# kezakool/flair-for-aigle

Measured on AMD Instinct MI355X. Metric: 512x512x5 tiles/sec (train fwd+bwd+AdamW), U-Net ResNet-34, 19 classes, higher is better.
Workload: dtype bf16; 1 GPU; synthetic 512x512x5 tiles, 19-class U-Net (ResNet-34 encoder), batch 32 per GPU, train step (BASELINE.json configs[1]); global_batch=32, tile=512, parallelism=dp1

## Files before the change

### flair-for-aigle_amd/csrc/conv_igemm.hip

```cpp
#include "ffa_gfx950.h"

#include <stdlib.h>

#ifndef FFA_CONV_READS_FIRST
#define FFA_CONV_READS_FIRST 0
#endif

#ifndef FFA_CONV_TRACE
#define FFA_CONV_TRACE 0
#endif
#if FFA_CONV_TRACE
#ifndef FFA_CONV_TRACE_FIRST
#define FFA_CONV_TRACE_FIRST 0
#endif
__device__ long long ffa_conv_trace_buf[64 * 256];
#define FFA_TRACE(slot_)                                                                    \
  if (trace_on) {                                                                           \
    if (trace_n < 256) ffa_conv_trace_buf[(blockIdx.x - FFA_CONV_TRACE_FIRST) * 256 + trace_n] = (long long)(slot_) << 56 | (__builtin_readcyclecounter() & 0xFFFFFFFFFFFFFFLL); \
    ++trace_n;                                                                              \
  }
#else
#define FFA_TRACE(slot_)
#endif

// ... 647 lines not shown
      const bool ok = (i < G::H_PIECES) && vy >= 0 && vx >= 0 && vy < a.Hi && vx < a.Wi;
      ho[k] = ok ? (((t.b * a.Hi + vy) * a.Wi + vx) * a.Ci * EB + hh * 16) : -1;
    }
  };

  int vb = next_valid(blockIdx.x);
  if (vb >= total_vb) return;
  TileId cur = decode(vb);
  int hoff[G::NHP];
  halo_offsets(cur, hoff);
  const unsigned char* in_b = static_cast<const unsigned char*>(a.in);
  const unsigned char* w_all = static_cast<const unsigned char*>(a.w);
  const unsigned char* w_b = w_all + (size_t)cur.cb * total_chunks * slab;

  ffa_u32x4 wregA[G::NWP], wregB[G::NWP];
  ffa_u32x4 hreg[G::NHP];
  ffa_f32x16 acc[G::MT][G::NT];

#define FFA_P_STORE_W(WR)                                                                  \
  {                                                                                        \
    _Pragma("unroll") for (int k = 0; k < G::NWP; ++k) {                                   \
      const int i = tid + k * G::NTHR;                                                     \
      if (k + 1 < G::NWP || G::W_PIECES % G::NTHR == 0 || i < G::W_PIECES) {               \
        const int row = i / (G::TAPS * 2), col = i % (G::TAPS * 2);                        \
        *reinterpret_cast<ffa_u32x4*>(sW + row * G::WP + col * 16) = WR[k];                \
      }                                                                                    \
    }                                                                                      \
  }
#define FFA_P_STORE_H(HO)                                                                  \
  {                                                                                        \
    _Pragma("unroll") for (int k = 0; k < G::NHP; ++k) {                                   \
      const int i = tid + k * G::NTHR;                                                     \
      if (k + 1 < G::NHP || G::H_PIECES % G::NTHR == 0 || i < G::H_PIECES)                 \
        *reinterpret_cast<ffa_u32x4*>(sIn + hlds0 + k * HLDS_STEP) = (HO[k] >= 0) ? hreg[k] : ffa_u32x4{0u, 0u, 0u, 0u}; \
    }                                                                                      \
  }

  {
    const ffa_u32x4* wsrc = reinterpret_cast<const ffa_u32x4*>(w_b);
#pragma unroll
    for (int k = 0; k < G::NWP; ++k) {
      const int i = tid + k * G::NTHR;
      wregA[k] = wsrc[(k + 1 < G::NWP || G::W_PIECES % G::NTHR == 0 || i < G::W_PIECES) ? i : 0];
    }
#pragma unroll
    for (int k = 0; k < G::NHP; ++k) hreg[k] = *reinterpret_cast<const ffa_u32x4*>(in_b + (unsigned)(hoff[k] >= 0 ? hoff[k] : 0));
    FFA_P_STORE_W(wregA)
    FFA_P_STORE_H(hoff)
    __syncthreads();
    const ffa_u32x4* wsrc1 = reinterpret_cast<const ffa_u32x4*>(w_b + slab);
#pragma unroll
    for (int k = 0; k < G::NWP; ++k) {
      const int i = tid + k * G::NTHR;
      wregA[k] = wsrc1[(k + 1 < G::NWP || G::W_PIECES % G::NTHR == 0 || i < G::W_PIECES) ? i : 0];
    }
  }

  constexpr int HJ = (HK >= 4) ? 1 : 0;
  while (true) {
    const int nvb = next_valid(vb + gridDim.x);
    const bool has_next = nvb < total_vb;
    const TileId nxt = decode(has_next ? nvb : vb);
    const unsigned char* w_n = w_all + (size_t)nxt.cb * total_chunks * slab;

#pragma unroll
    for (int mt = 0; mt < G::MT; ++mt)
#pragma unroll
      for (int nt = 0; nt < G::NT; ++nt)
#pragma unroll
        for (int r = 0; r < 16; ++r) acc[mt][nt][r] = 0.f;

    for (int c0 = 0; c0 < total_chunks; c0 += HK) {
      const bool last_group = (c0 + HK >= total_chunks);
      const bool cross = last_group && has_next;
      const unsigned char* hbase = in_b + (last_group ? (has_next ? 0 : c0 * 32) : (c0 + HK) * 32);
      if (cross) halo_offsets(nxt, hoff);
#pragma unroll
      for (int j = 0; j < HK; ++j) {
        const int c = c0 + j;
        const unsigned char* wp = (c + 2 < total_chunks) ? w_b + (size_t)(c + 2) * slab
                                  : (has_next ? w_n + (size_t)(c + 2 - total_chunks) * slab
                                              : w_b + (size_t)(total_chunks - 1) * slab);
        const ffa_u32x4* wsrc = reinterpret_cast<const ffa_u32x4*>(wp);
        auto issue = [&](int tap) __attribute__((always_inline)) {
#pragma unroll
          for (int k = 0; k < G::NWP; ++k) {
            if (k % G::TAPS != tap) continue;
            const int i = tid + k * G::NTHR;
            const ffa_u32x4 v = wsrc[(k + 1 < G::NWP || G::W_PIECES % G::NTHR == 0 || i < G::W_PIECES) ? i : 0];
            if (j & 1) wregA[k] = v;
            else wregB[k] = v;
          }
          if (j == HJ) {
#pragma unroll
            for (int k = 0; k < G::NHP; ++k) {
              if (k % G::TAPS != tap) continue;
              hreg[k] = *reinterpret_cast<const ffa_u32x4*>(hbase + (unsigned)(hoff[k] >= 0 ? hoff[k] : 0));
            }
          }
        };
        {
          const int sub = j * 32;
          ffa_u32x4 af[2][G::MT], bf[2][G::NT];
#pragma unroll
          for (int mt = 0; mt < G::MT; ++mt) af[0][mt] = *reinterpret_cast<const ffa_u32x4*>(sW + aoff[mt]);
#pragma unroll
          for (int nt = 0; nt < G::NT; ++nt) bf[0][nt] = *reinterpret_cast<const ffa_u32x4*>(sIn + boff[nt] + sub);
#pragma unroll
          for (int tap = 0; tap < G::TAPS; ++tap) {
            const int cu = tap & 1, nx = cu ^ 1;
            __builtin_amdgcn_sched_barrier(0);
            issue(tap);
            if (tap + 1 < G::TAPS) {
              const int r1 = (tap + 1) / KW, s1 = (tap + 1) % KW;
#pragma unroll
              for (int mt = 0; mt < G::MT; ++mt)
                af[nx][mt] = *reinterpret_cast<const ffa_u32x4*>(sW + aoff[mt] + (tap + 1) * 32);
#pragma unroll
              for (int nt = 0; nt < G::NT; ++nt)
                bf[nx][nt] = *reinterpret_cast<const ffa_u32x4*>(sIn + boff[nt] + sub + (r1 * G::IW + s1) * G::PP);
            }
#pragma unroll
            for (int mt = 0; mt < G::MT; ++mt)
#pragma unroll
              for (int nt = 0; nt < G::NT; ++nt) Mma<T>::run(af[cu][mt], bf[cu][nt], acc[mt][nt]);
            {
              constexpr int NM = G::MT * G::NT;
              const int NR = (tap + 1 < G::TAPS) ? G::MT + G::NT : 0;
              int NV = 0;
#pragma unroll
              for (int k = 0; k < G::NWP; ++k) NV += (k % G::TAPS == tap) ? 1 : 0;
              if (j == HJ) {
#pragma unroll
                for (int k = 0; k < G::NHP; ++k) NV += (k % G::TAPS == tap) ? 1 : 0;
              }
              constexpr int PER = (sizeof(T) == 2) ? 1 : 4;
#pragma unroll
              for (int i = 0; i < NM; ++i) {
                __builtin_amdgcn_sched_group_barrier(0x008, PER, 0);
                if (i < NR) __builtin_amdgcn_sched_group_barrier(0x100, 1, 0);
                if (i < NV) __builtin_amdgcn_sched_group_barrier(0x020, 1, 0);
              }
#pragma unroll
              for (int i = NM; i < G::MT + G::NT; ++i)
                if (i < NR) __builtin_amdgcn_sched_group_barrier(0x100, 1, 0);
#pragma unroll
              for (int i = NM; i < NM + 4; ++i)
                if (i < NV) __builtin_amdgcn_sched_group_barrier(0x020, 1, 0);
            }
          }
          __builtin_amdgcn_sched_barrier(0);
        }
        __syncthreads();
        if (c + 1 < total_chunks || has_next) {
          if (j & 1) FFA_P_STORE_W(wregB)
          else FFA_P_STORE_W(wregA)
          if (j == HK - 1) FFA_P_STORE_H(hoff)
          __syncthreads();
        }
      }
    }

    {
      T* out = static_cast<T*>(a.out);
      const T* res = static_cast<const T*>(a.res);
      const int co_wave = cur.cb * BCO;
      constexpr int NCH = (G::MT == 2) ? 32 : 16;
      float st[2 * NCH];
      const bool want_stats = a.stats != nullptr;
#pragma unroll
      for (int i = 0; i < 2 * NCH; ++i) st[i] = 0.f;
#pragma unroll
      for (int nt = 0; nt < G::NT; ++nt) {
        const int n = wpx * G::WAVE_PX + nt * 32 + rho;
        const int oy = cur.oy0 + n / TW, ox = cur.ox0 + n % TW;
        if (oy >= a.Ho || ox >= a.Wo) continue;
        const long long pix = ((long long)(cur.b * a.Ho + oy) * a.Wo + ox) * (long long)a.Co;
#pragma unroll
        for (int g = 0; g < 4; ++g) {
          if (G::MT == 2) {
            const int c0 = co_wave + 16 * g + 8 * half;
            if (c0 >= a.Co) continue;
            float v[8];
#pragma unroll
            for (int i = 0; i < 4; ++i) {
              v[i] = acc[0][nt][4 * g + i];
              v[4 + i] = acc[G::MT - 1][nt][4 * g + i];
            }
            if (a.bias) {
#pragma unroll
              for (int i = 0; i < 8; ++i) v[i] += a.bias[c0 + i];
            }
            if (res) {
              float rv[8];
              ffa_load8<T>(res + pix + c0, rv);
#pragma unroll
              for (int i = 0; i < 8; ++i) v[i] += rv[i];
            }
            if (a.relu) {
#pragma unroll
              for (int i = 0; i < 8; ++i) v[i] = fmaxf(v[i], 0.f);
            }
            ffa_store8<T>(out + pix + c0, v);
            if (want_stats) {
#pragma unroll
              for (int i = 0; i < 8; ++i) {
                const float r = (EB == 2) ? ffa_bf16_bits_to_f32(ffa_f32_to_bf16_bits(v[i])) : v[i];
                st[g * 8 + i] += r;
                st[NCH + g * 8 + i] = __builtin_fmaf(r, r, st[NCH + g * 8 + i]);
              }
            }
          } else {
            const int c0 = co_wave + 8 * g + 4 * half;
            if (c0 >= a.Co) continue;
            float v[4];
#pragma unroll
            for (int i = 0; i < 4; ++i) v[i] = acc[0][nt][4 * g + i];
            if (a.bias) {
#pragma unroll
              for (int i = 0; i < 4; ++i) v[i] += a.bias[c0 + i];
            }
            if (res) {
#pragma unroll
              for (int i = 0; i < 4; ++i) v[i] += ffa_load_elem<T>(res + pix + c0 + i);
            }
            if (a.relu) {
#pragma unroll
              for (int i = 0; i < 4; ++i) v[i] = fmaxf(v[i], 0.f);
            }
            if (EB == 2) {
              uint2 u;
              u.x = ffa_pack_bf16x2(v[0], v[1]);
              u.y = ffa_pack_bf16x2(v[2], v[3]);
              *reinterpret_cast<uint2*>(out + pix + c0) = u;
            } else {
              *reinterpret_cast<float4*>(out + pix + c0) = make_float4(v[0], v[1], v[2], v[3]);
            }
            if (want_stats) {
#pragma unroll
              for (int i = 0; i < 4; ++i) {
                const float r = (EB == 2) ? ffa_bf16_bits_to_f32(ffa_f32_to_bf16_bits(v[i])) : v[i];
                st[g * 4 + i] += r;
                st[NCH + g * 4 + i] = __builtin_fmaf(r, r, st[NCH + g * 4 + i]);
              }
            }
          }
        }
      }
      if (want_stats) {
#pragma unroll
        for (int bit = 4; bit >= 0; --bit) {
          const int n = (2 * NCH) >> (4 - bit);
          if (n > 2) {
            const bool up = (rho >> bit) & 1;
#pragma unroll
            for (int jj = 0; jj < NCH; ++jj) {
              if (jj < n / 2) {
                float lo = st[jj], hi = st[jj + n / 2];
                asm volatile("" : "+v"(lo), "+v"(hi));
                const float keep = up ? hi : lo;
                const float send = up ? lo : hi;
                st[jj] = keep + __shfl_xor(send, 1 << bit, 64);
              }
            }
          } else {
            st[0] += __shfl_xor(st[0], 1 << bit, 64);
            st[1] += __shfl_xor(st[1], 1 << bit, 64);
          }
        }
        red[(wpx * 64 + lane) * 2 + 0] = st[0];
        red[(wpx * 64 + lane) * 2 + 1] = st[1];
        __syncthreads();
        constexpr int NOUT = (G::MT == 2) ? 128 : 64;
        if (tid < NOUT) {
          const int jj = tid & 1;
          const int ln = (G::MT == 2) ? (tid >> 1) : ((tid >> 1) * 2);
          float t = 0.f;
#pragma unroll
          for (int w = 0; w < WPX; ++w) t += red[(w * 64 + ln) * 2 + jj];
          const int r5 = ln & 31, hf = ln >> 5;
          const int which = r5 >> 4;
          int c;
          if (G::MT == 2) {
            const int L = (r5 & 15) * 2 + jj;
            c = cur.cb * BCO + 16 * (L >> 3) + 8 * hf + (L & 7);
          } else {
            const int L = ((r5 >> 1) & 7) * 2 + jj;
            c = cur.cb * BCO + 8 * (L >> 2) + 4 * hf + (L & 3);
          }
          if (c < a.Co) a.stats[((size_t)cur.pt * 2 + which) * a.Co + c] = t;
        }
        __syncthreads();
      }
    }
    if (!has_next) break;
    vb = nvb;
    cur = nxt;
    w_b = w_n;
  }
#undef FFA_P_STORE_W
#undef FFA_P_STORE_H
}


struct ConvPlan {
  int bco;
  int rg;
  int th, tw;
};

static int conv_rg(int kh) { return kh == 7 ? 1 : kh; }

static int conv_pref_bco(int kh, int kw, int stride, int cout) {
  if (kh == 3 && kw == 3 && stride == 1) return cout > 32 ? 64 : 32;
  return cout > 32 ? 64 : 32;
}

static bool conv_supported(int kh, int kw, int stride, int bco) {
  const bool shape = (kh == 3 && kw == 3 && (stride == 1 || stride == 2)) ||
                     (kh == 1 && kw == 1 && (stride == 1 || stride == 2)) || (kh == 7 && kw == 7 && stride == 2);
  if (!shape) return false;
  return bco == 64 || bco == 32;
}

static int conv_persist_grid(int dil, int c1_out, const void* bnx, int grid) {
  const char* pe = getenv("FFA_CONV_PERSIST");
  if ((pe && pe[0] == '0') || dil != 1 || c1_out != 0 || bnx != nullptr) return 0;
  const char* pm = getenv("FFA_CONV_PERSIST_MIN");
  const char* pg = getenv("FFA_CONV_PERSIST_GRID");
  const int min_grid = pm ? atoi(pm) : 0;
  int pgrid = pg ? atoi(pg) : 512;
  pgrid = pgrid < 8 ? 8 : (pgrid / 8) * 8;
  if (grid <= min_grid) return 0;
  return pgrid < grid ? pgrid : grid;
}

template <typename T, int KH, int KW, int STRIDE, int RG, int BCO, int WCO, int WPX, int TH, int TW, int HK,
          bool UP = false>
static int launch_hk(const ConvArgs& a, hipStream_t stream) {
  const int grid = ffa_cdiv(a.npt, 8) * 8 * a.ncb;
  if constexpr (KH == 3 && KW == 3 && STRIDE == 1 && HK >= 2 && !UP && WCO == 1 && WPX == 4) {
    const int pgrid = conv_persist_grid(a.dil, a.c1_out, a.bnx, grid);
    if (pgrid > 0) {
      hipLaunchKernelGGL((conv3x3_persist_kernel<T, BCO, TH, TW, HK>), dim3(pgrid), dim3(256), 0, stream, a);
      return ffa_check_launch("conv3x3_persist");
    }
  }
  hipLaunchKernelGGL((conv_igemm_kernel<T, KH, KW, STRIDE, RG, BCO, WCO, WPX, TH, TW, HK, UP>), dim3(grid),
                     dim3(64 * WCO * WPX), 0, stream, a);
  return ffa_check_launch("conv_igemm");
}

template <typename T, int BCO, int TH, int TW>
static int launch_up(const ConvArgs& a, hipStream_t stream) {
  if (a.nchunks % 4 == 0) return launch_hk<T, 3, 3, 1, 3, BCO, 1, 4, TH, TW, 4, true>(a, stream);
  return launch_hk<T, 3, 3, 1, 3, BCO, 1, 4, TH, TW, 2, true>(a, stream);
}

template <typename T, int KH, int KW, int STRIDE, int RG, int BCO, int WCO, int WPX, int TH, int TW>
static int launch_cfg(const ConvArgs& a, hipStream_t stream) {
  if constexpr (KH == 3 && STRIDE == 1) {
    if (a.nchunks % 4 == 0) return launch_hk<T, KH, KW, STRIDE, RG, BCO, WCO, WPX, TH, TW, 4>(a, stream);
    if (a.nchunks % 2 == 0) return launch_hk<T, KH, KW, STRIDE, RG, BCO, WCO, WPX, TH, TW, 2>(a, stream);
  }
  return launch_hk<T, KH, KW, STRIDE, RG, BCO, WCO, WPX, TH, TW, 1>(a, stream);
}

template <typename T, int KH, int KW, int STRIDE, int RG>
static int launch_shape(const ConvArgs& a, const ConvPlan& p, hipStream_t stream) {
  const bool wide = (p.tw == 32);
#define FFA_CONV_CASE(BCO_, WCO_, WPX_)                                                      \
  if (p.bco == BCO_) {                                                                       \
    return wide ? launch_cfg<T, KH, KW, STRIDE, RG, BCO_, WCO_, WPX_, 8, 32>(a, stream)      \
                : launch_cfg<T, KH, KW, STRIDE, RG, BCO_, WCO_, WPX_, 16, 16>(a, stream);    \
  }
  FFA_CONV_CASE(64, 1, 4)
  FFA_CONV_CASE(32, 1, 4)
#undef FFA_CONV_CASE
  ffa_set_error("conv: no kernel for bco=%d", p.bco);
  return FFA_ERR_UNSUPPORTED;
}

template <typename T>
static int launch_dtype(const ConvArgs& a, int kh, int kw, int stride, const ConvPlan& p, hipStream_t stream) {
  if (kh == 3 && kw == 3 && stride == 1) return launch_shape<T, 3, 3, 1, 3>(a, p, stream);
  if (kh == 3 && kw == 3 && stride == 2) return launch_shape<T, 3, 3, 2, 3>(a, p, stream);
  if (kh == 1 && kw == 1 && stride == 1) return launch_shape<T, 1, 1, 1, 1>(a, p, stream);
  if (kh == 1 && kw == 1 && stride == 2) return launch_shape<T, 1, 1, 2, 1>(a, p, stream);
  if (kh == 7 && kw == 7 && stride == 2) return launch_shape<T, 7, 7, 2, 1>(a, p, stream);
  ffa_set_error("conv: unsupported kernel %dx%d stride %d", kh, kw, stride);
  return FFA_ERR_UNSUPPORTED;
}

extern "C" int ffa_conv_block_co(int kh, int kw, int stride, int cout) {
  const int bco = conv_pref_bco(kh, kw, stride, cout);
  return conv_supported(kh, kw, stride, bco) ? bco : FFA_ERR_UNSUPPORTED;
}

extern "C" int ffa_conv_plan(int dtype, int kh, int kw, int stride, int cout, int ci_pitch, int allow_ring) {
  const int bco = ffa_conv_block_co(kh, kw, stride, cout);
  if (bco < 0) return bco;
  {
    const char* t = getenv("FFA_STEM");
    if ((allow_ring & 4) && !(t && t[0] == '0') && ffa_stem_eligible(dtype, kh, kw, stride, cout, ci_pitch))
      return 64 | FFA_BCO_STEM;
  }
  {
    const char* t = getenv("FFA_THIN");
    if ((allow_ring & 2) && !(t && t[0] == '0') && ffa_thin_eligible(dtype, kh, kw, stride, cout, ci_pitch))
      return (cout <= 16 ? 16 : 32) | FFA_BCO_THIN | (ci_pitch == 32 ? FFA_BCO_THIN32 : 0);
  }
  allow_ring &= 1;
  const char* e = getenv("FFA_RING");
  const int eb = (dtype == FFA_BF16) ? 2 : 4;
  const bool on = (dtype == FFA_BF16) ? !(e && e[0] == '0') : (e && e[0] == '1');
  if (allow_ring && on && kh == 3 && kw == 3 && stride == 1 && cout >= 64 && (ci_pitch * eb) % 64 == 0)
    return 64 | FFA_BCO_RING;
  return bco;
}

extern "C" int ffa_conv_row_group(int kh) { return conv_rg(kh); }

static int conv2d_impl(int dtype, const void* in, const void* w_packed, const float* bias, const void* residual,
                       void* out, float* stat_partials, int B, int Hi, int Wi, int Ci, int Ho, int Wo, int Co,
                       int co_rows, int bco, int kh, int kw, int stride, int pad, int dil, int relu,
                       hipStream_t stream, void* out2 = nullptr, int c1_out = 0, const void* bnx = nullptr,
                       const float* bn_sc = nullptr, const float* bn_sh = nullptr) {
  FFA_REQUIRE(dtype == FFA_BF16 || dtype == FFA_F32, "conv: bad dtype %d", dtype);
  FFA_REQUIRE(in && w_packed && out, "conv: null pointer");
  FFA_REQUIRE(B > 0 && Hi > 0 && Wi > 0 && Ho > 0 && Wo > 0, "conv: bad dims");
  FFA_REQUIRE(Ci % 16 == 0 && Co % 8 == 0, "conv: channel pitch must be a multiple of 16 (in) / 8 (out), got %d/%d", Ci, Co);
  FFA_REQUIRE(dil == 1 || dil == 2, "conv: dil must be 1 or 2");
  FFA_REQUIRE(dil == 1 || stride == 1, "conv: zero-insertion input needs stride 1");
  FFA_REQUIRE((long long)B * Hi * Wi * Ci * (dtype == FFA_BF16 ? 2 : 4) < (1LL << 31),
              "conv: input tensor must be smaller than 2 GiB (32-bit piece offsets)");
  if (bco & FFA_BCO_STEM) {
    FFA_REQUIRE(dtype == FFA_BF16 && kh == 7 && kw == 7 && stride == 2 && pad == 3 && dil == 1 && c1_out == 0 && bnx == nullptr &&
                    residual == nullptr,
                "conv: a stem-layout operand serves the bf16 7x7 stride-2 pad-3 convolution only (no residual input)");
    return ffa_stem_conv7x7(in, w_packed, bias, out, stat_partials, B, Hi, Wi, Ci, Ho, Wo, Co, relu, stream);
  }
  if (bco & FFA_BCO_THIN) {
    FFA_REQUIRE(dtype == FFA_BF16 && kh == 3 && kw == 3 && stride == 1 && pad == 1 && dil == 1 && Hi == Ho && Wi == Wo &&
                    bnx == nullptr,
                "conv: a thin-layout operand serves bf16 3x3 stride-1 pad-1 convolutions only");
    if (c1_out > 0) {
      FFA_REQUIRE(c1_out == Co && out2 == nullptr && !stat_partials, "conv: thin pooled form takes C2 = 0 only");
      return ffa_thin_conv3x3(in, w_packed, nullptr, nullptr, out, nullptr, B, Hi, Wi, Ci, Co, co_rows, 0, 0, 1, stream);
    }
    return ffa_thin_conv3x3(in, w_packed, bias, residual, out, stat_partials, B, Hi, Wi, Ci, Co, co_rows, relu, 0, 0,
                            stream);
  }
  if (bco & FFA_BCO_RING) {
    FFA_REQUIRE(kh == 3 && kw == 3 && stride == 1 && pad == 1 && dil == 1 && Hi == Ho && Wi == Wo && c1_out == 0 &&
                    bnx == nullptr,
                "conv: a ring-layout operand serves plain 3x3 stride-1 pad-1 convolutions only");
    return ffa_ring_conv3x3(dtype, in, w_packed, bias, residual, out, stat_partials, nullptr, nullptr, B, Hi, Wi, Ci, Co,
                            co_rows, relu, stream);
  }
  if (!conv_supported(kh, kw, stride, bco)) {
    ffa_set_error("conv: unsupported kernel %dx%d stride %d block %d", kh, kw, stride, bco);
    return FFA_ERR_UNSUPPORTED;
  }
  ConvPlan p;
  p.bco = bco;
  p.rg = conv_rg(kh);
  p.tw = (Wo >= 32) ? 32 : 16;
  p.th = (Wo >= 32) ? 8 : 16;
  FFA_REQUIRE(co_rows % p.bco == 0, "conv: packed weight rows %d not a multiple of block %d", co_rows, p.bco);
  ConvArgs a;
  a.in = in;
  a.w = w_packed;
  a.out = out;
  a.bias = bias;
  a.stats = stat_partials;
  a.in2 = nullptr;
  a.c1_bytes = 0;
  a.out2 = out2;
  a.c1_out = c1_out;
  a.bnx = bnx;
  a.bn_sc = bn_sc;
  a.bn_sh = bn_sh;
  a.res = residual;
  a.B = B; a.Hi = Hi; a.Wi = Wi; a.Ci = Ci;
  a.Ho = Ho; a.Wo = Wo; a.Co = Co;
  a.pad = pad; a.dil = dil; a.relu = relu;
  const int eb = (dtype == FFA_BF16) ? 2 : 4;
  a.nchunks = Ci * eb / 32;
  a.tiles_x = ffa_cdiv(Wo, p.tw);
  a.tiles_y = ffa_cdiv(Ho, p.th);
  a.npt = B * a.tiles_x * a.tiles_y;
  a.ncb = co_rows / p.bco;
  if (dtype == FFA_BF16) return launch_dtype<ffa_bf16>(a, kh, kw, stride, p, stream);
  return launch_dtype<float>(a, kh, kw, stride, p, stream);
}

extern "C" int ffa_conv2d(int dtype, const void* in, const void* w_packed, const float* bias, const void* residual,
                          void* out, int B, int Hi, int Wi, int Ci, int Ho, int Wo, int Co, int co_rows, int bco,
                          int kh, int kw, int stride, int pad, int dil, int relu, hipStream_t stream) {
  return conv2d_impl(dtype, in, w_packed, bias, residual, out, nullptr, B, Hi, Wi, Ci, Ho, Wo, Co, co_rows, bco, kh, kw,
                     stride, pad, dil, relu, stream);
}

extern "C" int ffa_conv2d_pro(int dtype, const void* in, const void* w_packed, const float* bias, const void* residual,
                              void* out, float* stat_partials, const float* pro_scale, const float* pro_shift, int B,
                              int H, int W, int Ci, int Co, int co_rows, int bco, int relu, int up, hipStream_t stream) {
  FFA_REQUIRE(dtype == FFA_BF16 && in && w_packed && out && pro_scale && pro_shift, "conv_pro: bad arguments");
  if (bco & FFA_BCO_THIN)
    return ffa_thin_conv3x3_pro(in, w_packed, bias, residual, out, stat_partials, pro_scale, pro_shift, B, H, W, Ci, Co,
                                co_rows, relu, up, 0, stream);
  if ((bco & FFA_BCO_RING) && !up)
    return ffa_ring_conv3x3(dtype, in, w_packed, bias, residual, out, stat_partials, pro_scale, pro_shift, B, H, W, Ci, Co,
                            co_rows, relu, stream);
  ffa_set_error("conv_pro: no prologue kernel for this operand layout (bco 0x%x, up %d)", bco, up);
  return FFA_ERR_UNSUPPORTED;
}

extern "C" int ffa_conv2d_bnbwd(int dtype, const void* in, const void* w_packed, const void* residual, void* out,
                                float* stat_partials, const void* bnx, const float* bn_scale, const float* bn_shift,
                                int B, int Hi, int Wi, int Ci, int Ho, int Wo, int Co, int co_rows, int bco, int kh,
                                int kw, int stride, int pad, int dil, hipStream_t stream) {
  FFA_REQUIRE(stat_partials && bnx && bn_scale && bn_shift, "conv_bnbwd: null pointer");
  return conv2d_impl(dtype, in, w_packed, nullptr, residual, out, stat_partials, B, Hi, Wi, Ci, Ho, Wo, Co, co_rows,
                     bco, kh, kw, stride, pad, dil, 0, stream, nullptr, 0, bnx, bn_scale, bn_shift);
}

static long long conv_stat_rows_igemm(int B, int Ho, int Wo) {
  const int tw = (Wo >= 32) ? 32 : 16, th = (Wo >= 32) ? 8 : 16;
  return (long long)B * ffa_cdiv(Wo, tw) * ffa_cdiv(Ho, th);
}
extern "C" long long ffa_conv_stat_rows(int B, int Ho, int Wo, int co_rows, int bco) {
  if (bco & FFA_BCO_STEM) return ffa_stem_stat_rows(B, Ho, Wo);
  if (bco & FFA_BCO_THIN) return ffa_thin_stat_rows(B, Ho, Wo, (bco & FFA_BCO_THIN32) ? 32 : 16);
  if (bco & FFA_BCO_RING) return ffa_ring_stat_rows(B, Ho, Wo, co_rows);
  return conv_stat_rows_igemm(B, Ho, Wo);
}

extern "C" int ffa_conv_is_persistent(int dtype, int B, int Ho, int Wo, int Ci, int co_rows, int bco, int kh, int kw,
                                      int stride, int dil) {
  if (!(kh == 3 && kw == 3 && stride == 1) || bco <= 0 || co_rows % bco != 0) return 0;
  const int nchunks = Ci * (dtype == FFA_BF16 ? 2 : 4) / 32;
  if (nchunks % 2 != 0) return 0;
  if (bco & (FFA_BCO_RING | FFA_BCO_THIN | FFA_BCO_STEM)) return 0;
  const int npt = (int)conv_stat_rows_igemm(B, Ho, Wo);
  return conv_persist_grid(dil, 0, nullptr, ffa_cdiv(npt, 8) * 8 * (co_rows / bco)) > 0 ? 1 : 0;
}

extern "C" int ffa_conv2d_stats(int dtype, const void* in, const void* w_packed, const float* bias,
                                const void* residual, void* out, float* stat_partials, int B, int Hi, int Wi, int Ci,
                                int Ho, int Wo, int Co, int co_rows, int bco, int kh, int kw, int stride, int pad,
                                int dil, int relu, hipStream_t stream) {
  FFA_REQUIRE(stat_partials, "conv_stats: null statistics buffer");
  return conv2d_impl(dtype, in, w_packed, bias, residual, out, stat_partials, B, Hi, Wi, Ci, Ho, Wo, Co, co_rows, bco,
                     kh, kw, stride, pad, dil, relu, stream);
}

extern "C" int ffa_conv2d_upcat(int dtype, const void* lo, const void* skip, const void* w_packed, const float* bias,
                                void* out, float* stat_partials, int B, int Hl, int Wl, int C1, int C2, int Co,
                                int co_rows, int bco, int relu, hipStream_t stream) {
  FFA_REQUIRE(dtype == FFA_BF16 || dtype == FFA_F32, "conv_upcat: bad dtype %d", dtype);
  FFA_REQUIRE(lo && w_packed && out && (skip || C2 == 0), "conv_upcat: null pointer");
  FFA_REQUIRE(B > 0 && Hl > 0 && Wl > 0 && C1 > 0 && C2 >= 0 && C1 % 16 == 0 && C2 % 16 == 0 && Co % 8 == 0,
              "conv_upcat: bad dims");
  const int eb = (dtype == FFA_BF16) ? 2 : 4;
  const int Hi = 2 * Hl, Wi = 2 * Wl, Ci = C1 + C2;
  if (bco & FFA_BCO_THIN) {
    if (C2 != 0 || dtype != FFA_BF16) {
      ffa_set_error("conv_upcat: a thin-layout operand takes the skip-less form only");
      return FFA_ERR_UNSUPPORTED;
    }
    return ffa_thin_conv3x3(lo, w_packed, bias, nullptr, out, stat_partials, B, Hi, Wi, C1, Co, co_rows, relu, 1, 0, stream);
  }
  FFA_REQUIRE((long long)B * Hi * Wi * (C1 > C2 ? C1 : C2) * eb < (1LL << 31),
              "conv_upcat: source tensors must be smaller than 2 GiB (32-bit piece offsets)");
  if (!conv_supported(3, 3, 1, bco) || co_rows % bco != 0) {
    ffa_set_error("conv_upcat: unsupported block %d / rows %d", bco, co_rows);
    return FFA_ERR_UNSUPPORTED;
  }
  const int nchunks = Ci * eb / 32;
  const int hk = (nchunks % 4 == 0) ? 4 : (nchunks % 2 == 0 ? 2 : 1);
  if (hk == 1 || (C1 * eb) % (hk * 32) != 0) {
    ffa_set_error("conv_upcat: C1 = %d does not cover whole %d-byte channel groups", C1, hk * 32);
    return FFA_ERR_UNSUPPORTED;
  }
  ConvArgs a;
  a.in = lo;
  a.in2 = skip;
  a.c1_bytes = C1 * eb;
  a.out2 = nullptr;
  a.c1_out = 0;
  a.bnx = nullptr;
  a.bn_sc = a.bn_sh = nullptr;
  a.w = w_packed;
  a.out = out;
  a.bias = bias;
  a.stats = stat_partials;
  a.res = nullptr;
  a.B = B; a.Hi = Hi; a.Wi = Wi; a.Ci = Ci;
  a.Ho = Hi; a.Wo = Wi; a.Co = Co;
  a.pad = 1; a.dil = 1; a.relu = relu;
  a.nchunks = nchunks;
  const int tw = (Wi >= 32) ? 32 : 16, th = (Wi >= 32) ? 8 : 16;
  a.tiles_x = ffa_cdiv(Wi, tw);
  a.tiles_y = ffa_cdiv(Hi, th);
  a.npt = B * a.tiles_x * a.tiles_y;
  a.ncb = co_rows / bco;
#define FFA_UP_CASE(T_)                                                         \
  if (bco == 64) return (tw == 32) ? launch_up<T_, 64, 8, 32>(a, stream) : launch_up<T_, 64, 16, 16>(a, stream); \
  return (tw == 32) ? launch_up<T_, 32, 8, 32>(a, stream) : launch_up<T_, 32, 16, 16>(a, stream);
  if (dtype == FFA_BF16) { FFA_UP_CASE(ffa_bf16) }
  FFA_UP_CASE(float)
#undef FFA_UP_CASE
}

extern "C" int ffa_conv2d_dgrad_upcat(int dtype, const void* dy, const void* w_packed_t, void* dlo, void* dskip, int B,
                                      int Ho, int Wo, int Cdy, int C1, int C2, int co_rows, int bco,
                                      hipStream_t stream) {
  FFA_REQUIRE(dy && w_packed_t && dlo && (dskip || C2 == 0), "dgrad_upcat: null pointer");
  FFA_REQUIRE(Ho % 2 == 0 && Wo % 2 == 0 && C1 > 0 && C2 >= 0 && C1 % 8 == 0 && C2 % 8 == 0, "dgrad_upcat: bad dims");
  if (bco & FFA_BCO_THIN) {
    if (C2 != 0) {
      ffa_set_error("dgrad_upcat: a thin-layout operand takes the skip-less form only");
      return FFA_ERR_UNSUPPORTED;
    }
    return conv2d_impl(dtype, dy, w_packed_t, nullptr, nullptr, dlo, nullptr, B, Ho, Wo, Cdy, Ho, Wo, C1, co_rows, bco, 3,
                       3, 1, 1, 1, 0, stream, nullptr, C1);
  }
  if (C1 % bco != 0) {
    ffa_set_error("dgrad_upcat: C1 = %d is not a multiple of the %d-row block", C1, bco);
    return FFA_ERR_UNSUPPORTED;
  }
  return conv2d_impl(dtype, dy, w_packed_t, nullptr, nullptr, dlo, nullptr, B, Ho, Wo, Cdy, Ho, Wo, C1 + C2, co_rows,
                     bco, 3, 3, 1, 1, 1, 0, stream, dskip, C1);
}

#if FFA_CONV_TRACE
extern "C" int ffa_conv_trace_read(long long* host_dst, int n) {
  if (n > 64 * 256) n = 64 * 256;
  hipDeviceSynchronize();
  return (int)hipMemcpyFromSymbol(host_dst, HIP_SYMBOL(ffa_conv_trace_buf), (size_t)n * sizeof(long long));
}
extern "C" int ffa_conv_trace_clear() {
  static long long zeros[64 * 256];
  return (int)hipMemcpyToSymbol(HIP_SYMBOL(ffa_conv_trace_buf), zeros, sizeof(zeros));
}
#endif
```

Measured before the change: 2393 tiles/s.

## Add parity-decomposed dgrad kernel for dilated stride-2 backward convolutions

Adds a specialised kernel for the data-gradient of stride-2 convolutions, which reach this path as dilation-2 stride-1 convolutions. The kernel splits output pixels into four parity classes so each class multiplies only against the taps that land on nonzero input, instead of running the full 3x3 (or 1x1) tap set over a zero-dilated input. For 1x1 it writes the other three parity pixels directly, as the residual or as zero. The path is on by default and can be turned off with an environment variable. It adds a new launch path with its own tiling and bounds checks, which carries some correctness risk.

```diff
diff --git a/flair-for-aigle_amd/csrc/conv_igemm.hip b/flair-for-aigle_amd/csrc/conv_igemm.hip
--- a/flair-for-aigle_amd/csrc/conv_igemm.hip
+++ b/flair-for-aigle_amd/csrc/conv_igemm.hip
@@ -973,6 +973,307 @@
 #undef FFA_P_STORE_H
 }
 
+struct ParityArgs {
+  const void* in;
+  const void* w;
+  void* out;
+  const void* res;
+  int B, Hi, Wi, Ci;
+  int Ho, Wo, Co;
+  int ngroups;
+  int ncb;
+  int first[5];
+  int tiles_x[2], tiles_y[2];
+};
+
+template <int KH, int TH, int TW, int PA, int PB>
+struct ParityGeom {
+  static constexpr int KK = KH * KH;
+  static constexpr int NR = PA ? 2 : 1, NS = PB ? 2 : 1;
+  static constexpr int NTAPS = NR * NS;
+  static constexpr int IH = TH + PA, IW = TW + PB;
+  static constexpr int PP = 4 * 32 + 16;
+  static constexpr int H_PIECES = IH * IW * 8;
+  static constexpr int NHP = (H_PIECES + 255) / 256;
+  static constexpr int WP = 4 * NTAPS * 32 + 16;
+  static constexpr int NWP = 64 * 4 * NTAPS * 2 / 256;
+  static constexpr int W_ROWS_PER_K = 256 / (8 * NTAPS);
+  static constexpr int HALO_BYTES = IH * IW * PP;
+  static constexpr int LDS_BYTES = HALO_BYTES + 64 * WP;
+  static_assert(KH == 3 || (KH == 1 && PA == 0 && PB == 0), "1x1: only class (0, 0) has a tap");
+  static_assert(TH * TW == 256 && (TW & (TW - 1)) == 0, "4 waves x 64 pixels");
+};
+
+template <int KH, int TH, int TW, int PA, int PB>
+__device__ __forceinline__ void dgrad_parity_body(const ParityArgs& a, int lb, unsigned char* smem) {
+  using G = ParityGeom<KH, TH, TW, PA, PB>;
+  using T = ffa_bf16;
+  unsigned char* sIn = smem;
+  unsigned char* sW = smem + G::HALO_BYTES;
+
+  const int tiles_x = a.tiles_x[PB], tiles_y = a.tiles_y[PA];
+  const int npt = a.B * tiles_x * tiles_y;
+  const int xcd = lb & 7;
+  const int jb = lb >> 3;
+  const int pt = (jb / a.ncb) * 8 + xcd;
+  const int cb = jb % a.ncb;
+  if (pt >= npt) return;
+  const int tx = pt % tiles_x;
+  const int t2 = pt / tiles_x;
+  const int ty = t2 % tiles_y;
+  const int b = t2 / tiles_y;
+  const int py0 = ty * TH, px0 = tx * TW;
+
+  const int tid = threadIdx.x;
+#if FFA_CONV_TRACE
+  const bool trace_on = (tid == 0 && (int)blockIdx.x >= FFA_CONV_TRACE_FIRST && (int)blockIdx.x < FFA_CONV_TRACE_FIRST + 64);
+  int trace_n = 0;
+#endif
+  FFA_TRACE(0)
+  const int lane = tid & 63;
+  const int wpx = tid >> 6;
+  const int rho = lane & 31;
+  const int half = lane >> 5;
+
+  int aoff[2], boff[2];
+#pragma unroll
+  for (int mt = 0; mt < 2; ++mt) aoff[mt] = (mt * 32 + rho) * G::WP + half * 16;
+#pragma unroll
+  for (int nt = 0; nt < 2; ++nt) {
+    const int n = wpx * 64 + nt * 32 + rho;
+    boff[nt] = ((n / TW) * G::IW + (n % TW)) * G::PP + half * 16;
+  }
+
+  ffa_f32x16 acc[2][2];
+#pragma unroll
+  for (int mt = 0; mt < 2; ++mt)
+#pragma unroll
+    for (int nt = 0; nt < 2; ++nt)
+#pragma unroll
+      for (int r = 0; r < 16; ++r) acc[mt][nt][r] = 0.f;
+
+  int hoff[G::NHP];
+#pragma unroll
+  for (int k = 0; k < G::NHP; ++k) {
+    const int i = tid + k * 256;
+    const int q = i >> 3, hh = i & 7;
+    const int vy = py0 + q / G::IW, vx = px0 + q % G::IW;
+    const bool ok = i < G::H_PIECES && vy < a.Hi && vx < a.Wi;
+    hoff[k] = ok ? (((b * a.Hi + vy) * a.Wi + vx) * a.Ci * 2 + hh * 16) : -1;
+  }
+  const int hlds0 = (tid >> 3) * G::PP + (tid & 7) * 16;
+  const int wrem = tid % (8 * G::NTAPS);
+  const int wrow = tid / (8 * G::NTAPS);
+  const int wj = wrem / (2 * G::NTAPS), wt = (wrem >> 1) % G::NTAPS, wh = wrem & 1;
+  const int wtap = (KH == 1) ? 0 : (PA ? 2 * (wt / G::NS) : 1) * 3 + (PB ? 2 * (wt % G::NS) : 1);
+  const int woff0 = (wj * 64 + wrow) * (G::KK * 32) + wtap * 32 + wh * 16;
+  const int wlds0 = wrow * G::WP + (wj * G::NTAPS + wt) * 32 + wh * 16;
+
+  const unsigned char* in_b = static_cast<const unsigned char*>(a.in);
+  const size_t wgroup = (size_t)4 * 64 * G::KK * 32;
+  const unsigned char* w_b = static_cast<const unsigned char*>(a.w) + (size_t)cb * a.ngroups * wgroup;
+
+  ffa_u32x4 wreg[G::NWP], hreg[G::NHP];
+  auto load_group = [&](int g) __attribute__((always_inline)) {
+    const unsigned char* wsrc = w_b + (size_t)g * wgroup + woff0;
+#pragma unroll
+    for (int k = 0; k < G::NWP; ++k)
+      wreg[k] = *reinterpret_cast<const ffa_u32x4*>(wsrc + k * (G::W_ROWS_PER_K * G::KK * 32));
+    const unsigned char* hsrc = in_b + g * 128;
+#pragma unroll
+    for (int k = 0; k < G::NHP; ++k) {
+      ffa_u32x4 v = ffa_u32x4{0u, 0u, 0u, 0u};
+      if (hoff[k] >= 0) v = *reinterpret_cast<const ffa_u32x4*>(hsrc + (unsigned)hoff[k]);
+      hreg[k] = v;
+    }
+  };
+  auto store_group = [&]() __attribute__((always_inline)) {
+#pragma unroll
+    for (int k = 0; k < G::NWP; ++k)
+      *reinterpret_cast<ffa_u32x4*>(sW + wlds0 + k * (G::W_ROWS_PER_K * G::WP)) = wreg[k];
+#pragma unroll
+    for (int k = 0; k < G::NHP; ++k) {
+      if (k + 1 < G::NHP || G::H_PIECES % 256 == 0 || tid + k * 256 < G::H_PIECES)
+        *reinterpret_cast<ffa_u32x4*>(sIn + hlds0 + k * (32 * G::PP)) = hreg[k];
+    }
+  };
+
+  T* __restrict__ out = static_cast<T*>(a.out);
+  const T* __restrict__ res = static_cast<const T*>(a.res);
+  long long pix[2];
+  int oyx[2][2];
+#pragma unroll
+  for (int nt = 0; nt < 2; ++nt) {
+    const int n = wpx * 64 + nt * 32 + rho;
+    const int oy = 2 * (py0 + n / TW) + PA, ox = 2 * (px0 + n % TW) + PB;
+    oyx[nt][0] = oy;
+    oyx[nt][1] = ox;
+    pix[nt] = (oy < a.Ho && ox < a.Wo) ? ((long long)(b * a.Ho + oy) * a.Wo + ox) * (long long)a.Co + cb * 64 + 8 * half : -1;
+  }
+  const int cleft = a.Co - (cb * 64 + 8 * half);
+  uint4 rown[2][4];
+  auto unpack8 = [](const uint4& u, float(&v)[8]) __attribute__((always_inline)) {
+    v[0] = __uint_as_float(u.x << 16); v[1] = __uint_as_float(u.x & 0xffff0000u);
+    v[2] = __uint_as_float(u.y << 16); v[3] = __uint_as_float(u.y & 0xffff0000u);
+    v[4] = __uint_as_float(u.z << 16); v[5] = __uint_as_float(u.z & 0xffff0000u);
+    v[6] = __uint_as_float(u.w << 16); v[7] = __uint_as_float(u.w & 0xffff0000u);
+  };
+
+  load_group(0);
+  store_group();
+  __syncthreads();
+  FFA_TRACE(1)
+  for (int g = 0; g < a.ngroups; ++g) {
+    const bool more = g + 1 < a.ngroups;
+    if (more) {
+      load_group(g + 1);
+    } else if (res) {
+#pragma unroll
+      for (int nt = 0; nt < 2; ++nt)
+#pragma unroll
+        for (int q = 0; q < 4; ++q) {
+          rown[nt][q] = make_uint4(0u, 0u, 0u, 0u);
+          if (pix[nt] >= 0 && 16 * q < cleft) rown[nt][q] = *reinterpret_cast<const uint4*>(res + pix[nt] + 16 * q);
+        }
+    }
+    FFA_TRACE(2)
+#pragma unroll
+    for (int j = 0; j < 4; ++j) {
+#pragma unroll
+      for (int t = 0; t < G::NTAPS; ++t) {
+        ffa_u32x4 af[2], bf[2];
+#pragma unroll
+        for (int mt = 0; mt < 2; ++mt)
+          af[mt] = *reinterpret_cast<const ffa_u32x4*>(sW + aoff[mt] + (j * G::NTAPS + t) * 32);
+#pragma unroll
+        for (int nt = 0; nt < 2; ++nt)
+          bf[nt] = *reinterpret_cast<const ffa_u32x4*>(sIn + boff[nt] + j * 32 + ((t / G::NS) * G::IW + t % G::NS) * G::PP);
+#pragma unroll
+        for (int mt = 0; mt < 2; ++mt)
+#pragma unroll
+          for (int nt = 0; nt < 2; ++nt) Mma<T>::run(af[mt], bf[nt], acc[mt][nt]);
+      }
+    }
+    FFA_TRACE(3)
+    if (more) {
+      __syncthreads();
+      FFA_TRACE(4)
+      store_group();
+      FFA_TRACE(5)
+      __syncthreads();
+      FFA_TRACE(6)
+    }
+  }
+
+#pragma unroll
+  for (int nt = 0; nt < 2; ++nt) {
+    if (pix[nt] < 0) continue;
+#pragma unroll
+    for (int g = 0; g < 4; ++g) {
+      if (16 * g >= cleft) continue;
+      float v[8];
+#pragma unroll
+      for (int i = 0; i < 4; ++i) {
+        v[i] = acc[0][nt][4 * g + i];
+        v[4 + i] = acc[1][nt][4 * g + i];
+      }
+      if (res) {
+        float rv[8];
+        unpack8(rown[nt][g], rv);
+#pragma unroll
+        for (int i = 0; i < 8; ++i) v[i] += rv[i];
+      }
+      ffa_store8<T>(out + pix[nt] + 16 * g, v);
+    }
+  }
+  if constexpr (KH == 1) {
+#pragma unroll
+    for (int nt = 0; nt < 2; ++nt) {
+      if (pix[nt] < 0) continue;
+      uint4 rq[3][4];
+      long long p2[3];
+#pragma unroll
+      for (int d = 1; d < 4; ++d) {
+        const bool ok = oyx[nt][0] + (d >> 1) < a.Ho && oyx[nt][1] + (d & 1) < a.Wo;
+        p2[d - 1] = ok ? pix[nt] + ((long long)(d >> 1) * a.Wo + (d & 1)) * (long long)a.Co : -1;
+#pragma unroll
+        for (int g = 0; g < 4; ++g) {
+          rq[d - 1][g] = make_uint4(0u, 0u, 0u, 0u);
+          if (res && ok && 16 * g < cleft) rq[d - 1][g] = *reinterpret_cast<const uint4*>(res + p2[d - 1] + 16 * g);
+        }
+      }
+#pragma unroll
+      for (int d = 0; d < 3; ++d) {
+        if (p2[d] < 0) continue;
+#pragma unroll
+        for (int g = 0; g < 4; ++g) {
+          if (16 * g >= cleft) continue;
+          float z[8];
+          unpack8(rq[d][g], z);
+#pragma unroll
+          for (int i = 0; i < 8; ++i) z[i] += 0.f;
+          ffa_store8<T>(out + p2[d] + 16 * g, z);
+        }
+      }
+    }
+  }
+  FFA_TRACE(7)
+}
+
+template <int KH, int TH, int TW>
+__global__ void __launch_bounds__(256, 2) conv_dgrad_parity_kernel(ParityArgs a) {
+  __shared__ __align__(16) unsigned char smem[ParityGeom<KH, TH, TW, KH == 3, KH == 3>::LDS_BYTES];
+  const int bid = blockIdx.x;
+  if constexpr (KH == 1) {
+    dgrad_parity_body<1, TH, TW, 0, 0>(a, bid, smem);
+  } else {
+    if (bid < a.first[1]) dgrad_parity_body<3, TH, TW, 1, 1>(a, bid, smem);
+    else if (bid < a.first[2]) dgrad_parity_body<3, TH, TW, 1, 0>(a, bid - a.first[1], smem);
+    else if (bid < a.first[3]) dgrad_parity_body<3, TH, TW, 0, 1>(a, bid - a.first[2], smem);
+    else dgrad_parity_body<3, TH, TW, 0, 0>(a, bid - a.first[3], smem);
+  }
+}
+
+
+static bool conv_parity_eligible(int dtype, int kh, int kw, int stride, int pad, int dil, int bco, int Ci, int relu,
+                                 const float* bias, const float* stats, int c1_out, const void* bnx) {
+  const char* e = getenv("FFA_DGRAD_PARITY");
+  if (e && e[0] == '0') return false;
+  if (dtype != FFA_BF16 || dil != 2 || stride != 1 || bco != 64 || relu || bias || stats || c1_out != 0 || bnx) return false;
+  if (!((kh == 3 && kw == 3 && pad == 1) || (kh == 1 && kw == 1 && pad == 0))) return false;
+  return (Ci * 2) % 128 == 0;
+}
+
+static int launch_parity(const void* in, const void* w_packed, const void* residual, void* out, int B, int Hi, int Wi,
+                         int Ci, int Ho, int Wo, int Co, int co_rows, int kh, hipStream_t stream) {
+  ParityArgs a;
+  a.in = in; a.w = w_packed; a.out = out; a.res = residual;
+  a.B = B; a.Hi = Hi; a.Wi = Wi; a.Ci = Ci;
+  a.Ho = Ho; a.Wo = Wo; a.Co = Co;
+  a.ngroups = Ci * 2 / 128;
+  a.ncb = co_rows / 64;
+  const bool wide = (Wo + 1) / 2 >= 32;
+  const int tw = wide ? 32 : 16, th = wide ? 8 : 16;
+  for (int p = 0; p < 2; ++p) {
+    a.tiles_x[p] = ffa_cdiv((Wo + 1 - p) / 2, tw);
+    a.tiles_y[p] = ffa_cdiv((Ho + 1 - p) / 2, th);
+  }
+  int grid = 0;
+  for (int s = 0; s < 4; ++s) {
+    const int pa = 1 - s / 2, pb = 1 - s % 2;
+    a.first[s] = grid;
+    if (kh == 3 || s == 3) grid += ffa_cdiv(B * a.tiles_x[pb] * a.tiles_y[pa], 8) * 8 * a.ncb;
+  }
+  a.first[4] = grid;
+  if (grid == 0) return FFA_OK;
+#define FFA_PARITY_CASE(KH_)                                                                                       \
+  if (wide) hipLaunchKernelGGL((conv_dgrad_parity_kernel<KH_, 8, 32>), dim3(grid), dim3(256), 0, stream, a);       \
+  else hipLaunchKernelGGL((conv_dgrad_parity_kernel<KH_, 16, 16>), dim3(grid), dim3(256), 0, stream, a);
+  if (kh == 3) { FFA_PARITY_CASE(3) }
+  else { FFA_PARITY_CASE(1) }
+#undef FFA_PARITY_CASE
+  return ffa_check_launch("conv_dgrad_parity");
+}
 
 struct ConvPlan {
   int bco;
@@ -1139,6 +1440,8 @@
   p.tw = (Wo >= 32) ? 32 : 16;
   p.th = (Wo >= 32) ? 8 : 16;
   FFA_REQUIRE(co_rows % p.bco == 0, "conv: packed weight rows %d not a multiple of block %d", co_rows, p.bco);
+  if (conv_parity_eligible(dtype, kh, kw, stride, pad, dil, bco, Ci, relu, bias, stat_partials, c1_out, bnx))
+    return launch_parity(in, w_packed, residual, out, B, Hi, Wi, Ci, Ho, Wo, Co, co_rows, kh, stream);
   ConvArgs a;
   a.in = in;
   a.w = w_packed;
```

New measurement: 2414 tiles/s, median of 6. No clear change (+0.9%).
